# Atticuszz/GsplatLoc

Measured on AMD Instinct MI355X. Metric: Gaussians/s fwd+bwd @1M splats 1200x680, higher is better.
Workload: dtype f32

## Files before the change

### gsplatloc_amd/csrc/gsloc_common.h

```cpp
#pragma once
#include <hip/hip_runtime.h>
#include <stdint.h>

#include "../../include/gsloc_hip.h"

#define GSL_WAVE 64
#define GSL_ALPHA_MAX 0.999f
#define GSL_ALPHA_MIN (1.0f / 255.0f)
#define GSL_T_STOP 1e-4f
#define GSL_LOG2E 1.4426950408889634f

#define GSL_CHECK_LAUNCH()                                   \
  do {                                                       \
    hipError_t e__ = hipGetLastError();                      \
    if (e__ != hipSuccess) return GSL_ERR_HIP;               \
  } while (0)

namespace gsl {

int zero_u32(void* p, size_t n_dwords, hipStream_t st);

struct M3 {
  float m[9];
  __device__ __forceinline__ float& operator()(int r, int c) { return m[r * 3 + c]; }
// ... 42 lines not shown
  M3 R = quat_to_rotmat(q[0], q[1], q[2], q[3]);
  M3 M;
#pragma unroll
  for (int i = 0; i < 3; ++i)
#pragma unroll
    for (int j = 0; j < 3; ++j) M(i, j) = R(i, j) * s[j];
  return mul_bt(M, M);
}

struct Cam {
  M3 R;
  float t[3];
  float fx, fy, cx, cy;
};

__device__ __forceinline__ Cam load_cam(const float* __restrict__ V, const float* __restrict__ K) {
  Cam c;
#pragma unroll
  for (int i = 0; i < 3; ++i) {
#pragma unroll
    for (int j = 0; j < 3; ++j) c.R(i, j) = V[i * 4 + j];
    c.t[i] = V[i * 4 + 3];
  }
  c.fx = K[0]; c.fy = K[4]; c.cx = K[2]; c.cy = K[5];
  return c;
}

#define GSL_Q(arr, g) (arr)[(g)]
#ifndef GSL_NG
#define GSL_NG 4
#endif
#define GSL_HIT_SHIFT (32 - GSL_NG)
#define GSL_HIT_INDEX_MASK ((1u << GSL_HIT_SHIFT) - 1u)
#define GSL_CLAMP_DEPTH_WINDOW(nearp, farp)            \
  do {                                                 \
    if (!((nearp) >= 1.17549435e-38f)) (nearp) = 1.17549435e-38f; \
    if (!((farp) <= 3.40282347e+38f)) (farp) = 3.40282347e+38f;   \
  } while (0)
#define GSL_MAX_GAUSSIANS (1 << 26)
#ifndef GSL_XCD_SPANS
#define GSL_XCD_SPANS 0
#endif
__device__ __forceinline__ int xcd_span_item(int b, int n) {
#if GSL_XCD_SPANS
  const int x = b & 7, k = b >> 3, q = n >> 3, r = n & 7;
  return x * q + min(x, r) + k;
#else
  (void)n;
  return b;
#endif
}
#define GSL_TILE_OF_BLOCK() gsl::xcd_span_item((int)blockIdx.x, (int)gridDim.x)

__device__ __forceinline__ unsigned pack2h(float a, float b) {
  _Float16 ha = (_Float16)a, hb = (_Float16)b;
  return (unsigned)__builtin_bit_cast(unsigned short, ha) | ((unsigned)__builtin_bit_cast(unsigned short, hb) << 16);
}
__device__ __forceinline__ float h_lo(unsigned u) { return (float)__builtin_bit_cast(_Float16, (unsigned short)(u & 0xFFFFu)); }
__device__ __forceinline__ float h_hi(unsigned u) { return (float)__builtin_bit_cast(_Float16, (unsigned short)(u >> 16)); }

__device__ __forceinline__ void store_half_record(uint4* __restrict__ Qh, size_t i, float4 q0, float4 q1, float4 q2) {
  float rc = (q1.w > 0.f && q1.w < 6.0e4f) ? q1.w * 1.002f + 0.01f : q1.w;
  Qh[2 * i] = make_uint4(__float_as_uint(q0.x), __float_as_uint(q0.y), pack2h(q1.x, q1.y), pack2h(q1.z, rc));
  Qh[2 * i + 1] = make_uint4(pack2h(0.f, q0.w), pack2h(q2.x, q2.y), pack2h(q2.z, 0.f), __float_as_uint(q0.z));
}

// ... 349 lines not shown
```

### gsplatloc_amd/csrc/raster_g16.hip

```cpp
#include <stdlib.h>
#include <string.h>

#include "gsloc_common.h"

namespace gsl {

__device__ __forceinline__ float g16_sel(unsigned long long m, float t, float f) {
  float r;
  asm("v_cndmask_b32_e64 %0, %1, %2, %3" : "=v"(r) : "v"(f), "v"(t), "s"(m));
  return r;
}

#define G16_M_LO8 0x00FF00FF00FF00FFull
#define G16_M_B2 0x0F0F0F0F0F0F0F0Full
#define G16_M_B1 0x3333333333333333ull
#define G16_M_B0 0x5555555555555555ull

constexpr int G16_NG = GSL_NG;
constexpr int G16_GL = 64 / G16_NG;
static_assert(G16_NG == 4 || G16_NG == 8, "pixel groups are DPP rows or half rows");

__device__ __forceinline__ float row_scatter8(const float (&v)[8]) {
  float n0, n1, n2, n3, m0, m1;
  asm volatile(
// ... 48 lines not shown
      "v_add_f32_dpp %2, %6, %6 row_half_mirror row_mask:0xf bank_mask:0xf\n\t"
      "v_add_f32_dpp %3, %7, %7 row_half_mirror row_mask:0xf bank_mask:0xf\n\t"
      "v_add_f32_dpp %0, %8, %8 row_half_mirror row_mask:0xf bank_mask:0xa\n\t"
      "v_add_f32_dpp %1, %9, %9 row_half_mirror row_mask:0xf bank_mask:0xa\n\t"
      "v_add_f32_dpp %2, %10, %10 row_half_mirror row_mask:0xf bank_mask:0xa\n\t"
      "s_nop 1\n\t"
      : "=&v"(n0), "=&v"(n1), "=&v"(n2), "=&v"(n3)
      : "v"(v[0]), "v"(v[1]), "v"(v[2]), "v"(v[3]), "v"(v[4]), "v"(v[5]), "v"(v[6]));
  n0 += dpp_get<0x4E>(n0); n1 += dpp_get<0x4E>(n1); n2 += dpp_get<0x4E>(n2); n3 += dpp_get<0x4E>(n3);
  n0 += dpp_get<0xB1>(n0); n1 += dpp_get<0xB1>(n1); n2 += dpp_get<0xB1>(n2); n3 += dpp_get<0xB1>(n3);
  return make_float4(n0, n1, n2, n3);
}

__device__ __forceinline__ void half_scatter16(const float (&v)[16], float4& lo, float4& hi) {
  float a[8];
#pragma unroll
  for (int i = 0; i < 8; ++i) {
    float keep = g16_sel(G16_M_B2, v[i], v[i + 8]), send = g16_sel(G16_M_B2, v[i + 8], v[i]);
    a[i] = keep + dpp_get<0x141>(send);
  }
#pragma unroll
  for (int i = 0; i < 8; ++i) a[i] += dpp_get<0x4E>(a[i]);
#pragma unroll
  for (int i = 0; i < 8; ++i) a[i] += dpp_get<0xB1>(a[i]);
  lo = make_float4(a[0], a[1], a[2], a[3]);
  hi = make_float4(a[4], a[5], a[6], a[7]);
}

#ifdef GSL_G16_STATS
__device__ unsigned long long g16_stats[8];
#define G16_STAT(i, n) do { unsigned long long n__ = (unsigned long long)(n); if (lane == 0) atomicAdd(&g16_stats[i], n__); } while (0)
#else
#define G16_STAT(i, n) do { } while (0)
#endif

#ifndef GSL_QB
#define GSL_QB 64
#endif
#define GSL_QBS (GSL_QB + 1)
#ifndef GSL_Q_LCAP
#define GSL_Q_LCAP 24
#endif

template <int D, int CG>
struct QStage {
  static constexpr int NV = 6 + CG;
  static constexpr int NS = (NV <= 8) ? 8 : 16;
  static constexpr int A = 6 + D;
  static constexpr int LCAP = ((NS == 8) ? GSL_Q_LCAP : GSL_Q_LCAP / 2) * 4 / G16_NG;
  float4 s0[GSL_QBS];
  float4 s1[GSL_QBS];
  float4 s2[(D >= 3 && CG == D) ? GSL_QBS : 1];
  int32_t id[GSL_QBS];
  uint32_t posn[G16_NG / 4][GSL_QBS];
  alignas(16) float pair[G16_NG * LCAP * NS];
  uint8_t rlist[G16_NG][GSL_QBS + 4];
  uint8_t nzlist[64];
};

template <int D, int CG>
__device__ __forceinline__ void qraster_bwd_body(
    QStage<D, CG>& sb, const float4* __restrict__ Q0, const float4* __restrict__ Q1, const float4* __restrict__ Q2,
    const uint4* __restrict__ Qh, const int32_t* __restrict__ flatten_ids, float* __restrict__ vacc, long long rs,
    long long re, int lane, int quad, float px, float py, float tx0, float ty0, int bin_final, float T_init,
    float Bp_init, const float (&vc)[D], const uint32_t* __restrict__ qhits, int n_qhits) {
  constexpr bool RGB = D >= 3;
// ... 5 lines not shown
  constexpr int NG = G16_NG, GL = G16_GL;
  constexpr int PP = 12;
  static_assert(A <= PP && NG * LCAP * NS >= 64 * PP, "64 packed gradient rows reuse the pair slots");
  static_assert(GSL_QB < 127 && GSL_QB >= 64, "7-bit list positions with 127 reserved; a chunk appends up to 64 entries");
  const int grp = lane / GL, p = lane & (GL - 1);
  const float tcx = tx0 + 8.f, tcy = ty0 + 8.f;
  const float lx = px - tcx, ly = py - tcy;
  const float lxx = lx * lx, lxy = lx * ly, lyy = ly * ly;
  float T = T_init;
  float Bp = Bp_init;
  const int myslot = (NG == 8) ? (p >> 2) * (NS / 2) : ((NS == 8) ? (p >> 1) : p);
  const bool writer = (NG == 8) ? ((p & 3) == 0) : ((NS == 8) ? ((p & 1) == 0) : true);
  float* const mypair = &sb.pair[grp * LCAP * NS + myslot];
  uint8_t* const mylist = sb.rlist[grp];
  const unsigned long long lt = (1ull << lane) - 1ull;
  const float qx0 = tx0 + 8.f * (float)(quad & 1), qy0 = ty0 + 8.f * (float)(quad >> 1);
  int grp_final[NG];
  {
    int rf = bin_final;
    rf = max(rf, __shfl_xor(rf, 1, 64));
    rf = max(rf, __shfl_xor(rf, 2, 64));
    rf = max(rf, __shfl_xor(rf, 4, 64));
    if (GL == 16) rf = max(rf, __shfl_xor(rf, 8, 64));
#pragma unroll
    for (int g = 0; g < NG; ++g) grp_final[g] = __builtin_amdgcn_readlane(rf, GL * g);
  }
  if (lane == 0) {
    sb.s0[GSL_QB] = make_float4(0.f, 0.f, 0.f, 0.f);
    sb.s1[GSL_QB] = make_float4(0.f, 0.f, 0.f, 0.f);
    if (RGB && CG == D) sb.s2[GSL_QB] = make_float4(0.f, 0.f, 0.f, 0.f);
  }
  int pos = __builtin_amdgcn_readfirstlane(qhits ? n_qhits : (int)re);
  const int pos_end = __builtin_amdgcn_readfirstlane(qhits ? 0 : (int)rs);
  while (pos > pos_end) {
    int staged = 0;
    int cnt[NG];
#pragma unroll
    for (int g = 0; g < NG; ++g) cnt[g] = 0;
    __syncthreads();
    while (pos > pos_end && staged <= GSL_QB - 64) {
      long long idx = (long long)(pos - 1 - lane);
      bool in = idx >= (long long)pos_end;
      unsigned nib = 0;
      int gid = 0;
      float4 r0 = make_float4(0.f, 0.f, 0.f, 0.f), r1 = r0, r2 = r0;
      if (in) {
        if (qhits) {
          unsigned e = qhits[idx];
          nib = e >> GSL_HIT_SHIFT;
          idx = (long long)(e & GSL_HIT_INDEX_MASK);
          gid = flatten_ids[idx];
          load_record(Q0, Q1, Q2, Qh, gid, RGB && CG == D, r0, r1, r2);
        } else {
          gid = flatten_ids[idx];
          load_record(Q0, Q1, Q2, Qh, gid, RGB && CG == D, r0, r1, r2);
          if (r1.w >= 0.f) {
            float rr = r1.w * r1.w;
#pragma unroll
            for (int g = 0; g < NG; ++g) {
              const int b = (NG == 8) ? (g >> 1) : g;
              const float cy = (NG == 8) ? 2.f * (float)(g & 1) + 1.f : 2.f, hy = (NG == 8) ? 0.5f : 1.5f;
              float ex = fmaxf(fabsf(r0.x - (qx0 + 4.f * (float)(b & 1) + 2.f)) - 1.5f, 0.f);
              float ey = fmaxf(fabsf(r0.y - (qy0 + 4.f * (float)(b >> 1) + cy)) - hy, 0.f);
              bool h = (ex * ex + ey * ey <= rr) && ((int)idx <= grp_final[g]);
              nib |= (h ? 1u : 0u) << g;
            }
          }
        }
      }
      unsigned long long R = __ballot(nib != 0);
      int slot = staged + __popcll(R & lt);
      unsigned pack[NG / 4];
#pragma unroll
      for (int w = 0; w < NG / 4; ++w) pack[w] = 0x0FFFFFFFu;
#pragma unroll
      for (int g = 0; g < NG; ++g) {
        unsigned long long Bg = __ballot(nib & (1u << g));
        if (__builtin_amdgcn_inverse_ballot_w64(Bg)) {
          int q = cnt[g] + __popcll(Bg & lt);
          sb.rlist[g][q] = (uint8_t)slot;
          pack[g >> 2] ^= (127u ^ (unsigned)q) << (7 * (g & 3));
        }
        cnt[g] += __popcll(Bg);
      }
      if (__builtin_amdgcn_inverse_ballot_w64(R)) {
        sb.id[slot] = gid;
        sb.s0[slot] = r0;
        sb.s1[slot] = make_float4(r1.x * (0.5f * GSL_LOG2E), r1.y * GSL_LOG2E, r1.z * (0.5f * GSL_LOG2E),
                                  __int_as_float((int)idx));
        if (RGB && CG == D) sb.s2[slot] = r2;
#pragma unroll
        for (int w = 0; w < NG / 4; ++w) sb.posn[w][slot] = pack[w];
      }
      staged += __popcll(R);
      pos -= 64;
    }
    if (staged == 0) continue;
    int kmax = 0, cnt_tot = 0, cnt_my = 0;
#pragma unroll
    for (int g = 0; g < NG; ++g) {
      kmax = max(kmax, cnt[g]);
      cnt_tot += cnt[g];
      cnt_my = (grp == g) ? cnt[g] : cnt_my;
    }
    G16_STAT(6, kmax);
    G16_STAT(7, cnt_tot);
    (void)cnt_tot;
    for (int k = cnt_my + p; k < kmax + 3; k += GL) mylist[k] = (uint8_t)GSL_QB;
    __syncthreads();
    constexpr int NU = (GSL_QB + 63) / 64;
    float mo[NU][NV];
#pragma unroll
    for (int u = 0; u < NU; ++u)
#pragma unroll
      for (int q = 0; q < NV; ++q) mo[u][q] = 0.f;
    auto trip = [&](int t, const float4& c0, const float4& c1, float4& r, float4& r2) {
      float dx = c0.x - px, dy = c0.y - py;
      float sigma = fmaf(c1.y * dx, dy, fmaf(c1.x * dx, dx, c1.z * dy * dy));
      float vis = __builtin_amdgcn_exp2f(-sigma);
      float opv = c0.w * vis;
      float alpha = fminf(GSL_ALPHA_MAX, opv);
      unsigned long long validm = __ballot(__float_as_int(c1.w) <= bin_final) & __ballot(sigma >= 0.f) &
                                  __ballot(alpha >= GSL_ALPHA_MIN);
      G16_STAT(0, 1);
      r = make_float4(0.f, 0.f, 0.f, 0.f);
      r2 = r;
      if (validm) {
        G16_STAT(1, 1);
#ifdef GSL_G16_STATS
        {
          int groups_hit = 0;
          for (int g = 0; g < NG; ++g) groups_hit += ((validm >> (GL * g)) & ((1ull << GL) - 1ull)) != 0;
          G16_STAT(3, groups_hit);
        }
#endif
        G16_STAT(5, __popcll(validm));
        unsigned long long capm = __ballot(opv <= GSL_ALPHA_MAX);
        float am = g16_sel(validm, alpha, 0.f);
        float ra = __builtin_amdgcn_rcpf(1.f - am);
        T *= ra;
        float fac = am * T;
        float cdot;
// ... 29 lines not shown
          else r.x = row_scatter16(reinterpret_cast<const float(&)[16]>(val));
        }
      }
    };
    auto put = [&](float* dst, const float4& r, const float4& r2) {
      if (NG == 8) {
        *reinterpret_cast<float4*>(dst) = r;
        if (NS == 16) *reinterpret_cast<float4*>(dst + 4) = r2;
      } else {
        *dst = r.x;
      }
    };
    for (int k0 = 0; k0 < kmax; k0 += LCAP) {
      const int k1 = min(k0 + LCAP, kmax);
      int t0 = mylist[k0], t1 = mylist[k0 + 1];
      float4 qa0 = sb.s0[t0], qa1 = sb.s1[t0];
      float4 ra = make_float4(0.f, 0.f, 0.f, 0.f), ra2 = ra, rb = ra, rb2 = ra;
      float* dst = mypair;
      for (int k = k0; k < k1; k += 2) {
        if (k > k0 && writer) put(dst - NS, rb, rb2);
        const int t2 = mylist[k + 2];
        const float4 qb0 = sb.s0[t1], qb1 = sb.s1[t1];
        trip(t0, qa0, qa1, ra, ra2);
        if (writer) put(dst, ra, ra2);
        const int t3 = mylist[k + 3];
        qa0 = sb.s0[t2];
        qa1 = sb.s1[t2];
        trip(t1, qb0, qb1, rb, rb2);
        t0 = t2;
        t1 = t3;
        dst += 2 * NS;
      }
      if (writer) put(dst - NS, rb, rb2);
      __syncthreads();
#pragma unroll
      for (int u = 0; u < NU; ++u) {
        int slot = lane + 64 * u;
        if (slot < staged) {
#pragma unroll
          for (int w = 0; w < NG / 4; ++w) {
            unsigned pk = sb.posn[w][slot];
#pragma unroll
            for (int g4 = 0; g4 < 4; ++g4) {
              const int g = 4 * w + g4;
              const unsigned q = ((pk >> (7 * g4)) & 127u) - (unsigned)k0;
              if (q < (unsigned)LCAP) {
                const float4* src = reinterpret_cast<const float4*>(&sb.pair[(g * LCAP + q) * NS]);
                float4 a = src[0], c = src[1];
                mo[u][0] += a.x; mo[u][1] += a.y; mo[u][2] += a.z; mo[u][3] += a.w;
                mo[u][4] += c.x; mo[u][5] += c.y; mo[u][6] += c.z;
                if (NV > 7) mo[u][7 < NV ? 7 : 0] += c.w;
                if (NS == 16) {
                  float4 e = src[2];
                  if (NV > 8) mo[u][8 < NV ? 8 : 0] += e.x;
                  if (NV > 9) mo[u][9 < NV ? 9 : 0] += e.y;
                }
              }
            }
          }
        }
      }
      __syncthreads();
    }
#pragma unroll
    for (int u = 0; u < NU; ++u) {
      int slot = lane + 64 * u;
      bool nz = false;
      float row[A];
#pragma unroll
      for (int k = 0; k < A; ++k) row[k] = 0.f;
      if (slot < staged) {
        {
          unsigned bits = 0u;
#pragma unroll
          for (int k = 0; k < NV; ++k) bits |= __float_as_uint(mo[u][k]);
          nz = (bits << 1) != 0u;
        }
        if (nz) {
          float4 r0 = sb.s0[slot], r1 = sb.s1[slot];
          float X = r0.x - tcx, Y = r0.y - tcy, S = mo[u][0];
          float Sx = X * S - mo[u][1], Sy = Y * S - mo[u][2];
          float Sxx = X * (X * S - 2.f * mo[u][1]) + mo[u][3];
          float Sxy = X * (Y * S - mo[u][2]) - Y * mo[u][1] + mo[u][4];
          float Syy = Y * (Y * S - 2.f * mo[u][2]) + mo[u][5];
          float no = -r0.w;
          r1.x *= 2.f / GSL_LOG2E; r1.y *= 1.f / GSL_LOG2E; r1.z *= 2.f / GSL_LOG2E;
          row[0] = no * (r1.x * Sx + r1.y * Sy);
          row[1] = no * (r1.y * Sx + r1.z * Sy);
          row[2] = 0.5f * no * Sxx;
          row[3] = no * Sxy;
          row[4] = 0.5f * no * Syy;
          row[5] = S;
          if (CG == D) {
#pragma unroll
            for (int ch = 0; ch < D; ++ch) row[6 + ch] = mo[u][6 + ch];
          } else {
            row[6 + D - 1] = mo[u][6];
          }
        }
      }
      float* packed = sb.pair;
      if (nz) {
#pragma unroll
        for (int k = 0; k < A; ++k) packed[lane * PP + k] = row[k];
      }
      unsigned long long mask = __ballot(nz);
      int cntz = __popcll(mask);
      if (nz) sb.nzlist[__popcll(mask & lt)] = (uint8_t)lane;
      __syncthreads();
      constexpr int RPI = 64 / A;
      const int arow = lane / A, f = lane - arow * A;
      for (int i0 = 0; i0 < cntz; i0 += RPI) {
        int gi = i0 + arow;
        if (gi < cntz && arow < RPI) {
          int sl = sb.nzlist[gi];
          const unsigned off = ((unsigned)sb.id[sl + 64 * u] << 6) | ((unsigned)f << 2);
          atomicAdd(reinterpret_cast<float*>(reinterpret_cast<char*>(vacc) + off), packed[sl * PP + f]);
        }
      }
      __syncthreads();
    }
  }
}

template <int D, bool ED, int CG, bool LONG>
__device__ __forceinline__ void qraster_bwd_item(
    QStage<D, CG>& sb, int b, int n_items, const float4* __restrict__ Q0, const float4* __restrict__ Q1,
    const float4* __restrict__ Q2, int W, int H, int tile_w, int ty0, const int32_t* __restrict__ tile_offsets,
    const int32_t* __restrict__ flatten_ids, long long capacity, const float* __restrict__ render,
    const float* __restrict__ alphas, const int32_t* __restrict__ last_ids, const float* __restrict__ v_render,
    const float* __restrict__ v_alphas, float* __restrict__ vacc, int row0, int row1, const uint4* __restrict__ Qh,
    const uint32_t* __restrict__ isect_hits, int32_t* __restrict__ isect_hit_counts, int long_min, LongWs lw,
    int32_t* __restrict__ rgb_flag, int32_t* __restrict__ clear_counts, int32_t* __restrict__ clear_state) {
  if (!LONG && (CG == 1 || D == 3) && clear_counts && (b & 3) == 0 && threadIdx.x == 0) {
    clear_counts[ty0 * tile_w + (b >> 2)] = 0;
    if (b == 0 && clear_state) *clear_state = 0;
  }
  const int wi = LONG ? b : xcd_span_item(b, n_items);
  const int quad = wi & 3, item = wi >> 2;
  int tile, sgm = 0, gseg = 0;
  if (LONG) {
    gseg = item;
    if (gseg >= lw.n_seg[0]) return;
    tile = lw.seg_tile[gseg];
    sgm = lw.seg_idx[gseg];
    if (tile < 0) return;
  } else {
    tile = ty0 * tile_w + item;
  }
  int tyi = tile / tile_w, txi = tile - tyi * tile_w;
  int lane = threadIdx.x, grp = lane >> 4, p = lane & 15;
  int j = txi * 16 + (quad & 1) * 8 + (grp & 1) * 4 + (p & 3);
  int i = tyi * 16 + (quad >> 1) * 8 + (grp >> 1) * 4 + (p >> 2);
  float px = (float)j + 0.5f, py = (float)i + 0.5f;
  bool inside = (i < H) && (j < W) && (i >= row0) && (i < row1);
// ... 55 lines not shown
        for (int u = 0; u < 8; ++u) {
          if (stop || s0 + u >= nseg) continue;
          if (t8[u] == 2.f) { stop = true; continue; }
          float cc[4] = {c8[u].x, c8[u].y, c8[u].z, c8[u].w};
          float dot = 0.f;
#pragma unroll
          for (int k = 0; k < D; ++k) dot += vc[k] * cc[k];
          Bp_init += dot;
          if (t8[u] < 0.f) stop = true;
        }
      }
    }
  }
  const uint32_t* qh = nullptr;
  int nqh = 0;
  if (isect_hits) {
    long long ls = tile_offsets[tile], le = tile_offsets[tile + 1];
    if (le > capacity) le = capacity;
    if (LONG) {
      ls += (long long)sgm * GSL_SEG;
      le = min(ls + (long long)GSL_SEG, le);
      nqh = lw.seg_qcnt[gseg * 4 + quad];
    } else {
      nqh = isect_hit_counts[tile * 4 + quad];
    }
    qh = isect_hits + 4 * ls + (long long)quad * (le - ls);
    if (nqh == 0) return;
  }
  qraster_bwd_body<D, CG>(sb, Q0, Q1, Q2, Qh, flatten_ids, vacc, rs, re, lane, quad, px, py, (float)(txi * 16),
                          (float)(tyi * 16), bin_final, T_init, Bp_init, vc, qh, nqh);
}

template <int D, bool ED, int CG, bool LONG>
__global__ __launch_bounds__(64) void k_qraster_bwd(
    const float4* __restrict__ Q0, const float4* __restrict__ Q1, const float4* __restrict__ Q2, int W, int H,
    int tile_w, int ty0, const int32_t* __restrict__ tile_offsets, const int32_t* __restrict__ flatten_ids,
    long long capacity, const float* __restrict__ render, const float* __restrict__ alphas,
    const int32_t* __restrict__ last_ids, const float* __restrict__ v_render, const float* __restrict__ v_alphas,
    float* __restrict__ vacc, int row0, int row1, const uint4* __restrict__ Qh,
    const uint32_t* __restrict__ isect_hits, int32_t* __restrict__ isect_hit_counts, int long_min, LongWs lw,
    int32_t* __restrict__ rgb_flag, int32_t* __restrict__ clear_counts, int32_t* __restrict__ clear_state, int n_items) {
  __shared__ QStage<D, CG> sb;
  if (D == 4 && CG == D && rgb_flag && *rgb_flag == 0) return;
  for (int b = (int)blockIdx.x; b < n_items; b += (int)gridDim.x) {
    qraster_bwd_item<D, ED, CG, LONG>(sb, b, n_items, Q0, Q1, Q2, W, H, tile_w, ty0, tile_offsets, flatten_ids, capacity,
                                      render, alphas, last_ids, v_render, v_alphas, vacc, row0, row1, Qh, isect_hits,
                                      isect_hit_counts, long_min, lw, rgb_flag, clear_counts, clear_state);
    __syncthreads();
  }
}

}

#ifdef GSL_G16_STATS
extern "C" int gsl_g16_stats(unsigned long long* host_out, int reset) {
  if (hipMemcpyFromSymbol(host_out, HIP_SYMBOL(gsl::g16_stats), sizeof(unsigned long long) * 8) != hipSuccess) return -3;
  if (reset) {
    unsigned long long z[8] = {0};
    if (hipMemcpyToSymbol(HIP_SYMBOL(gsl::g16_stats), z, sizeof(z)) != hipSuccess) return -3;
  }
  return 0;
}
#endif

extern "C" int32_t* gsl_fused_bin_state(void* ws, int n_tiles);

extern "C" int gsl_g16_raster_bwd_launch(const float* Q0, const float* Q1, const float* Q2, int channels, int ed, int width,
                                         int height, int tile_w, int ty0, int ty1, const int32_t* tile_offsets,
                                         const int32_t* flatten_ids, int64_t capacity, const float* render,
                                         const float* alphas, const int32_t* last_ids, const float* v_render,
                                         const float* v_alphas, float* vacc, int row0, int row1, const void* Qh,
                                         const uint32_t* isect_hits, const int32_t* isect_hit_counts, int long_min,
                                         void* long_ws, int max_seg, int rgb_flag_index, void* clear_ws,
                                         void* stream) {
  hipStream_t st = (hipStream_t)stream;
  int nblk = long_ws ? max_seg : (ty1 - ty0) * tile_w;
  gsl::LongWs lw = gsl::long_ws_views(long_ws ? long_ws : (void*)0, long_ws ? max_seg : 0);
  const bool lng = long_ws != nullptr;
  int32_t* rgb_flag = isect_hit_counts ? const_cast<int32_t*>(isect_hit_counts) + rgb_flag_index : nullptr;
  int32_t* clear_counts = (int32_t*)clear_ws;
  int32_t* clear_state = clear_ws ? gsl_fused_bin_state(clear_ws, rgb_flag_index / 4) : nullptr;
#define CALL_Q(DD, EE, CC)                                                                                   \
  do {                                                                                                       \
    const int n_items = 4 * nblk;                                                                            \
    const int grid = ((DD) == 4 && (CC) == 4 && rgb_flag && n_items > 2048) ? 2048 : n_items;                \
    if (lng)                                                                                                 \
      hipLaunchKernelGGL((gsl::k_qraster_bwd<DD, EE, CC, true>), dim3(grid), dim3(64), 0, st, (const float4*)Q0, \
                         (const float4*)Q1, (const float4*)Q2, width, height, tile_w, ty0, tile_offsets,     \
                         flatten_ids, (long long)capacity, render, alphas, last_ids, v_render, v_alphas, vacc, \
                         row0, row1, (const uint4*)Qh, isect_hits, const_cast<int32_t*>(isect_hit_counts), long_min, lw, rgb_flag, clear_counts, clear_state, n_items);                   \
    else                                                                                                     \
      hipLaunchKernelGGL((gsl::k_qraster_bwd<DD, EE, CC, false>), dim3(grid), dim3(64), 0, st, (const float4*)Q0, \
// ... 16 lines not shown
```

### gsplatloc_amd/csrc/raster_px.hip

```cpp
#include "gsloc_common.h"
#include "loss_dev.h"
#include "sort_dev.h"

namespace gsl {

template <int D>
struct PStage {
  float4 s0[256];
  float4 s1[256];
  float4 s2[(D >= 3) ? 256 : 1];
  uint16_t qlist[4][256];
  int qcnt[4][4];
};

template <int SHIFT = 0, typename Stage>
__device__ __forceinline__ int compact_quadrants(Stage& sb, int tid, bool valid_rec, float x, float y, float r,
                                                 float tile_x0, float tile_y0) {
  int lane = tid & 63, wv = tid >> 6;
  unsigned long long B[4];
#pragma unroll
  for (int q = 0; q < 4; ++q) {
    float cx = tile_x0 + 4.f + 8.f * (float)(q & 1), cy = tile_y0 + 4.f + 8.f * (float)(q >> 1);
    B[q] = __ballot(valid_rec) & __ballot(fabsf(x - cx) <= r + 3.5f) & __ballot(fabsf(y - cy) <= r + 3.5f);
  }
  if (lane < 4) {
    unsigned long long b = lane == 0 ? B[0] : (lane == 1 ? B[1] : (lane == 2 ? B[2] : B[3]));
    sb.qcnt[wv][lane] = __popcll(b);
  }
  __syncthreads();
  unsigned long long lt = (1ull << lane) - 1ull;
#pragma unroll
  for (int q = 0; q < 4; ++q) {
    if ((B[q] >> lane) & 1ull) {
      int base = 0;
      for (int w = 0; w < wv; ++w) base += sb.qcnt[w][q];
      sb.qlist[q][base + __popcll(B[q] & lt)] = (uint16_t)(tid << SHIFT);
    }
// ... 52 lines not shown
  return r;
}

__device__ __forceinline__ int ffbl_raw(unsigned v) {
  int r;
  asm("v_ffbl_b32 %0, %1" : "=v"(r) : "v"(v));
  return r;
}

__device__ __forceinline__ float4 rec_at(const float4* arr, unsigned off) {
  return *reinterpret_cast<const float4*>(reinterpret_cast<const char*>(arr) + off);
}

__device__ __forceinline__ void box_range(float centre_rel, float r, int& lo, int& hi) {
  float l = ceilf(centre_rel - r), h = floorf(centre_rel + r);
  lo = (int)fmaxf(l, 0.f);
  hi = (int)fminf(h, 7.f);
}

template <int D, int MODE>
__device__ __forceinline__ void praster_walk(
    PStage<D>& sb, const float4* __restrict__ Q0, const float4* __restrict__ Q1, const float4* __restrict__ Q2,
    const uint4* __restrict__ Qh, const int32_t* __restrict__ flatten_ids, long long rs, long long re, int tid, float px,
    float py, int qx, int qy, int txi, int tyi, bool& done, float& T, float (&pix)[D], int& cur_idx,
    uint32_t* __restrict__ isect_hits, int& n_hits) {
  constexpr bool RGB = D >= 3;
  constexpr bool DEPTH = (D == 1) || (D == 4);
  const int lane = tid & 63, wv = tid >> 6;
  int nb = (int)((re - rs + 255) / 256);
  if (MODE == 1) isect_hits = nullptr;
  uint32_t* const qout = isect_hits ? isect_hits + 4 * rs + (long long)wv * (re - rs) : nullptr;
  n_hits = 0;
  unsigned long long DONE = __ballot(done);
  for (int b = 0; b < nb; ++b) {
    if (__syncthreads_and(DONE == ~0ull)) break;
    long long bstart = rs + (long long)b * 256;
    int bsize = (int)min((long long)256, re - bstart);
    float4 r0 = make_float4(0.f, 0.f, 0.f, 0.f), r1 = make_float4(0.f, 0.f, 0.f, -1.f);
    if (tid < bsize) {
      int g = flatten_ids[bstart + tid];
      float4 r2 = make_float4(0.f, 0.f, 0.f, 0.f);
      load_record(Q0, Q1, Q2, Qh, g, RGB && MODE == 0, r0, r1, r2);
      const float ca = r1.x * (0.5f * GSL_LOG2E), cb = r1.y * GSL_LOG2E, cc = r1.z * (0.5f * GSL_LOG2E);
      sb.s0[tid] = make_float4(r0.x, r0.y, ca, cb);
      if (RGB) {
        sb.s1[tid] = make_float4(cc, r0.w, r2.x, r2.y);
        sb.s2[tid] = make_float4(r2.z, r0.z, r1.w, 0.f);
      } else {
        sb.s1[tid] = make_float4(cc, r0.w, r0.z, r1.w);
      }
    } else {
      sb.s0[tid] = make_float4(0.f, 0.f, 0.f, 0.f);
      if (RGB) {
        sb.s1[tid] = make_float4(0.f, 0.f, 0.f, 0.f);
        sb.s2[tid] = make_float4(0.f, 0.f, -1.f, 0.f);
      } else {
        sb.s1[tid] = make_float4(0.f, 0.f, 0.f, -1.f);
      }
    }
    const int n = __builtin_amdgcn_readfirstlane(
        compact_quadrants<4>(sb, tid, tid < bsize, r0.x, r0.y, r1.w, (float)(txi * 16), (float)(tyi * 16)));
    for (int c = 0; c < n; c += 64) {
      if (DONE == ~0ull) break;
      int e = c + lane;
      int lox = 1, hix = 0, loy = 1, hiy = 0;
      if (e < n) {
        const unsigned off = sb.qlist[wv][e];
        float4 a0 = rec_at(sb.s0, off);
        float r = RGB ? rec_at(sb.s2, off).z : rec_at(sb.s1, off).w;
        box_range(a0.x - ((float)qx + 0.5f), r, lox, hix);
        box_range(a0.y - ((float)qy + 0.5f), r, loy, hiy);
      }
      unsigned mlo, mhi;
      pixel_masks<true>(lox, hix, loy, hiy, lane, mlo, mhi);
      mlo = sel_u32(DONE, 0u, mlo);
      mhi = sel_u32(DONE, 0u, mhi);
      unsigned cm[2] = {0u, 0u};
#pragma unroll
      for (int half = 0; half < 2; ++half) {
        unsigned m = half ? mhi : mlo;
        if (half) m = sel_u32(DONE, 0u, m);
        const uint16_t* const ql = &sb.qlist[wv][c + half * 32];
        unsigned long long ACT = __ballot(m != 0);
        if (ACT) do {
          const unsigned b0 = m & (0u - m);
          m ^= b0;
          const unsigned b1 = m & (0u - m);
          m ^= b1;
          const unsigned long long TWO = __ballot(b1 != 0u);
          const unsigned t0 = ql[ffbl_raw(b0)] & 0xFF0u;
          const unsigned t1 = ql[ffbl_raw(b1)] & 0xFF0u;
          float4 p0 = rec_at(sb.s0, t0), p1 = rec_at(sb.s1, t0);
          float4 u0 = rec_at(sb.s0, t1), u1 = rec_at(sb.s1, t1);
          float dx0 = p0.x - px, dy0 = p0.y - py, dx1 = u0.x - px, dy1 = u0.y - py;
          float sg0 = fmaf(p0.w * dx0, dy0, fmaf(p0.z * dx0, dx0, p1.x * dy0 * dy0));
          float sg1 = fmaf(u0.w * dx1, dy1, fmaf(u0.z * dx1, dx1, u1.x * dy1 * dy1));
          float al0 = fminf(GSL_ALPHA_MAX, p1.y * __builtin_amdgcn_exp2f(-sg0));
          float al1 = fminf(GSL_ALPHA_MAX, u1.y * __builtin_amdgcn_exp2f(-sg1));
          const unsigned long long OK0 = ACT & __ballot(sg0 >= 0.f) & __ballot(al0 >= GSL_ALPHA_MIN);
          const unsigned long long OK1 = TWO & __ballot(sg1 >= 0.f) & __ballot(al1 >= GSL_ALPHA_MIN);
          if (MODE == 1) {
            T *= 1.f - sel_f32(OK0, al0, 0.f);
            T *= 1.f - sel_f32(OK1, al1, 0.f);
            ACT = __ballot(m != 0);
            continue;
          }
          const unsigned long long S0R = __ballot(T * (1.f - al0) <= GSL_T_STOP);
          const unsigned long long STOP0 = OK0 & S0R, EFF0 = OK0 & ~S0R;
          const float a0 = sel_f32(EFF0, al0, 0.f);
          const float vis0 = a0 * T;
          const float T1 = T * (1.f - a0);
          const unsigned long long LIVE1 = OK1 & ~STOP0;
          const unsigned long long S1R = __ballot(T1 * (1.f - al1) <= GSL_T_STOP);
          const unsigned long long STOP1 = LIVE1 & S1R, EFF1 = LIVE1 & ~S1R;
          const float a1 = sel_f32(EFF1, al1, 0.f);
          const float vis1 = a1 * T1;
          T = T1 * (1.f - a1);
          if (RGB) {
            const float2 q20 = *reinterpret_cast<const float2*>(reinterpret_cast<const char*>(sb.s2) + t0);
            const float2 q21 = *reinterpret_cast<const float2*>(reinterpret_cast<const char*>(sb.s2) + t1);
            pix[0] += p1.z * vis0; pix[1] += p1.w * vis0; pix[2] += q20.x * vis0;
            if (DEPTH) pix[D - 1] += q20.y * vis0;
            pix[0] += u1.z * vis1; pix[1] += u1.w * vis1; pix[2] += q21.x * vis1;
            if (DEPTH) pix[D - 1] += q21.y * vis1;
          } else if (DEPTH) {
            pix[D - 1] += p1.z * vis0;
            pix[D - 1] += u1.z * vis1;
          }
          cm[half] |= sel_u32(EFF0, b0, 0u) | sel_u32(EFF1, b1, 0u);
          const unsigned long long STOPPED = STOP0 | STOP1;
          DONE |= STOPPED;
          m = sel_u32(STOPPED, 0u, m);
          ACT = __ballot(m != 0);
        } while (ACT);
      }
      {
        const bool any = (cm[0] | cm[1]) != 0u;
        const int pos = cm[1] ? 63 - __clz((int)cm[1]) : 31 - __clz((int)(cm[0] | 1u));
        const int tl = (sb.qlist[wv][c + pos] & 0xFF0u) >> 4;
        cur_idx = any ? (int)bstart + tl : cur_idx;
      }
      if (isect_hits) {
        unsigned rlo = group_or(cm[0]), rhi = group_or(cm[1]);
        unsigned nib = 0;
        unsigned long long Rm = 0ull;
#pragma unroll
        for (int g = 0; g < GSL_NG; ++g) {
          unsigned glo = (unsigned)__builtin_amdgcn_readlane((int)rlo, (64 / GSL_NG) * g);
          unsigned ghi = (unsigned)__builtin_amdgcn_readlane((int)rhi, (64 / GSL_NG) * g);
          unsigned long long gm = ((unsigned long long)ghi << 32) | glo;
          nib |= sel_u32(gm, 1u << g, 0u);
          Rm |= gm;
        }
        if (nib) qout[n_hits + __popcll(Rm & ((1ull << lane) - 1ull))] = (nib << GSL_HIT_SHIFT) | (unsigned)((int)bstart + (sb.qlist[wv][e] >> 4));
        n_hits += __popcll(Rm);
      }
    }
  }
  done = ((DONE >> lane) & 1ull) != 0ull;
}

struct TilePixel {
  int tyi, txi, qx, qy, i, j;
};
__device__ __forceinline__ TilePixel tile_pixel(int tile, int tile_w, int tid) {
  TilePixel t;
  int lane = tid & 63, wv = tid >> 6, grp = lane >> 4, pp = lane & 15;
  t.tyi = tile / tile_w;
  t.txi = tile - t.tyi * tile_w;
  t.qx = t.txi * 16 + (wv & 1) * 8;
  t.qy = t.tyi * 16 + (wv >> 1) * 8;
  t.j = t.qx + 4 * (grp & 1) + (pp & 3);
  t.i = t.qy + 4 * (grp >> 1) + (pp >> 2);
  return t;
}

struct FwdSort {
  uint64_t* bins;
  const int32_t* counts;
  int32_t* tile_offsets;
  int32_t* flatten_ids;
  int32_t* n_isects;
  int32_t* flags;
  int bin_cap;
  const int32_t* storage_of;
};
template <int SORT> struct FwdListPtr { typedef const int32_t* __restrict__ type; };
template <> struct FwdListPtr<2> { typedef const int32_t* type; };
template <> struct FwdListPtr<3> { typedef const int32_t* type; };

template <int D, bool ED, int SORT>
__global__ __launch_bounds__(256) __attribute__((amdgpu_waves_per_eu(SORT == 3 ? 4 : 6))) void k_praster_fwd(
    const float4* __restrict__ Q0, const float4* __restrict__ Q1, const float4* __restrict__ Q2, int W, int H,
    int tile_w, int ty0, typename FwdListPtr<SORT>::type tile_offsets, typename FwdListPtr<SORT>::type flatten_ids,
    long long capacity, float* __restrict__ render, float* __restrict__ alphas, int32_t* __restrict__ last_ids,
    int row0, int row1, const uint4* __restrict__ Qh, int32_t* __restrict__ clear_counts,
    int32_t* __restrict__ clear_state, uint32_t* __restrict__ isect_hits, int32_t* __restrict__ isect_hit_counts,
    int long_min, int n_tiles_total, FwdSort fs) {
  constexpr size_t SORT_BYTES = SORT ? (size_t)8 * 64 * (1 << SORT) * sizeof(uint64_t) : 0;
  constexpr size_t LDS_BYTES = sizeof(PStage<D>) > SORT_BYTES ? sizeof(PStage<D>) : SORT_BYTES;
  __shared__ __align__(16) unsigned char smem[LDS_BYTES];
  PStage<D>& sb = *reinterpret_cast<PStage<D>*>(smem);
  __shared__ int s_scan[5];
  int tile = ty0 * tile_w + GSL_TILE_OF_BLOCK();
  long long sorted_rs = 0, sorted_re = 0;
  if constexpr (SORT != 0) {
    const int tid = threadIdx.x, lane = tid & 63, wv = tid >> 6;
    int acc = prefix_count_share(fs.counts, tile, fs.bin_cap, tid);
#pragma unroll
    for (int o = 32; o >= 1; o >>= 1) acc += __shfl_xor(acc, o, 64);
    if (lane == 0) s_scan[wv] = acc;
    if (tid == 0) {
      int c_own = fs.counts[tile];
      s_scan[4] = min(c_own, fs.bin_cap);
      if (c_own > fs.bin_cap && fs.flags) { fs.flags[1] = 1; atomicMax(&fs.flags[2], c_own); }
    }
    __syncthreads();
    long long s0 = s_scan[0] + s_scan[1] + s_scan[2] + s_scan[3], e0 = s0 + s_scan[4];
    if (tid == 0) {
      fs.tile_offsets[tile] = (int32_t)s0;
      if (tile == n_tiles_total - 1) {
        fs.tile_offsets[tile + 1] = (int32_t)e0;
        if (fs.n_isects) fs.n_isects[0] = (int32_t)e0;
      }
    }
    if (e0 > capacity) e0 = capacity;
    int n = (int)max(e0 - s0, (long long)0);
    if (n > 256) {
      wg_sort_tile<SORT>(fs.bins + (size_t)tile * (size_t)fs.bin_cap, n, s0, tile, tid, reinterpret_cast<uint64_t*>(smem),
                         nullptr, fs.flatten_ids, nullptr, 0, fs.storage_of);
    } else if (n > 0 && wv == 0) {
      const uint64_t* src = fs.bins + (size_t)tile * (size_t)fs.bin_cap;
      uint64_t k[4];
#pragma unroll
      for (int r = 0; r < 4; ++r) k[r] = (lane * 4 + r < n) ? src[lane * 4 + r] : GSL_SORT_PAD;
      wave_sort_regs<2>(k, lane);
// ... 17 lines not shown
  bool inside = (i < H) && (j < W) && (i >= row0) && (i < row1);
  bool done = !inside;

  long long rs, re;
  if constexpr (SORT != 0) {
    rs = sorted_rs;
    re = sorted_re;
  } else {
    rs = tile_offsets[tile];
    re = tile_offsets[tile + 1];
    if (re > capacity) re = capacity;
    if (rs > re) rs = re;
    if (long_min > 0 && re - rs > long_min) return;
  }

  float T = 1.f;
  int cur_idx = 0;
  float pix[D];
#pragma unroll
  for (int k = 0; k < D; ++k) pix[k] = 0.f;
  int n_hits = 0;
  praster_walk<D, 0>(sb, Q0, Q1, Q2, Qh, flatten_ids, rs, re, tid, px, py, tp.qx, tp.qy, tp.txi, tp.tyi, done, T, pix,
                     cur_idx, isect_hits, n_hits);
  if (isect_hits && (tid & 63) == 0) isect_hit_counts[tile * 4 + (tid >> 6)] = n_hits;
  if (inside) {
    size_t pid = (size_t)i * W + j;
    float A = 1.f - T;
    alphas[pid] = A;
    if (ED) pix[D - 1] = pix[D - 1] / fmaxf(A, 1e-10f);
#pragma unroll
    for (int k = 0; k < D; ++k) render[pid * D + k] = pix[k];
    last_ids[pid] = cur_idx;
  }
}

template <int D, int PASS>
__global__ __launch_bounds__(256) void k_long_fwd(
    const float4* __restrict__ Q0, const float4* __restrict__ Q1, const float4* __restrict__ Q2, int W, int H,
    int tile_w, const int32_t* __restrict__ tile_offsets, const int32_t* __restrict__ flatten_ids, long long capacity,
    int row0, int row1, const uint4* __restrict__ Qh, uint32_t* __restrict__ isect_hits, LongWs w) {
  __shared__ PStage<D> sb;
  int g = blockIdx.x;
  if (g >= w.n_seg[0]) return;
  int tile = w.seg_tile[g], sgm = w.seg_idx[g];
  if (tile < 0) return;
  int tid = threadIdx.x;
  TilePixel tp = tile_pixel(tile, tile_w, tid);
  int i = tp.i, j = tp.j;
  float px = (float)j + 0.5f, py = (float)i + 0.5f;
  bool inside = (i < H) && (j < W) && (i >= row0) && (i < row1);
  long long rs = tile_offsets[tile], re = tile_offsets[tile + 1];
  if (re > capacity) re = capacity;
  long long ss = rs + (long long)sgm * GSL_SEG, se = min(ss + (long long)GSL_SEG, re);
  float pix[D];
#pragma unroll
  for (int k = 0; k < D; ++k) pix[k] = 0.f;
  size_t slot = (size_t)g * 256 + tid;
  if (PASS == 0) {
    float T = 1.f;
    int cur = 0;
    bool done = !inside;
    int nh = 0;
    praster_walk<D, 1>(sb, Q0, Q1, Q2, Qh, flatten_ids, ss, se, tid, px, py, tp.qx, tp.qy, tp.txi, tp.tyi, done, T, pix,
                       cur, nullptr, nh);
    w.P[slot] = T;
  } else {
// ... 274 lines not shown
          const float T1 = T0 * ra1;
          const float fac1 = a1 * T1;
          const float va1 = T1 * cd1 - ra1 * Bp0;
          T = T1;
          Bp = Bp0 + fac1 * cd1;
          if (__builtin_amdgcn_inverse_ballot_w64(OK0)) {
            float w = (opv0 <= GSL_ALPHA_MAX) ? vis0 * va0 : 0.f;
            int cc = j - tiny_origin(p0.x, p1.w), rr = i - tiny_origin(p0.y, p1.w);
            if ((unsigned)cc < 4u && (unsigned)rr < 4u)
              trec[(size_t)sb.id[t0] * 16 + rr * 4 + cc] = make_float2(w, fac0);
            else if (flags)
              flags[0] = 1;
          }
          if (__builtin_amdgcn_inverse_ballot_w64(OK1)) {
            float w = (opv1 <= GSL_ALPHA_MAX) ? vis1 * va1 : 0.f;
            int cc = j - tiny_origin(u0.x, u1.w), rr = i - tiny_origin(u0.y, u1.w);
            if ((unsigned)cc < 4u && (unsigned)rr < 4u)
              trec[(size_t)sb.id[t1] * 16 + rr * 4 + cc] = make_float2(w, fac1);
            else if (flags)
              flags[0] = 1;
          }
          ACT = __ballot(m != 0);
        } while (ACT);
      }
    }
  }
}


}

extern "C" int32_t* gsl_fused_bin_state(void* ws, int n_tiles);

extern "C" int gsl_tiny_raster_bwd(const float* Q0, const float* Q1, const float* Q2, int channels, int ed, int width,
                                   int height, int tile_w, int tile_h, int ty0, int ty1, const int32_t* tile_offsets,
                                   const int32_t* flatten_ids, int64_t capacity, const float* render,
                                   const float* alphas, const int32_t* last_ids, const float* v_render,
                                   const float* v_alphas, float* trec, float* vcT, int row0, int row1,
                                   int32_t* flags, int long_min, const float* loss_depth_gt, float depth_lambda,
                                   float edge_lambda, float* loss_partials, void* clear_ws, void* stream) {
  if (width <= 0 || height <= 0 || tile_w <= 0 || tile_h <= 0 || ty0 < 0 || ty1 > tile_h || ty0 > ty1 ||
      capacity < 0 || row0 < 0 || row0 > row1)
    return GSL_ERR_BAD_ARG;
  if (tile_w * 16 < width || tile_h * 16 < height) return GSL_ERR_BAD_ARG;
  if (!tile_offsets || !render || !alphas || !last_ids || !v_render || !v_alphas || !trec || !vcT)
    return GSL_ERR_BAD_ARG;
  if (ed && channels == 3) return GSL_ERR_BAD_ARG;
  const bool loss = loss_depth_gt != nullptr;
  if (loss && (!loss_partials || ty0 != 0 || ty1 != tile_h || row0 != 0 || row1 < height ||
               tile_w != (width + 15) / 16 || tile_h != (height + 15) / 16 || (channels != 1 && channels != 4)))
    return GSL_ERR_BAD_ARG;
  if (ty0 == ty1) return GSL_OK;
  if (capacity > 0 && (!Q0 || !Q1 || !flatten_ids || (channels >= 3 && !Q2))) return GSL_ERR_BAD_ARG;
  hipStream_t st = (hipStream_t)stream;
  int nblk = (ty1 - ty0) * tile_w;
  gsl::TinyLoss tl{loss_depth_gt, loss_partials, const_cast<float*>(v_render), depth_lambda, edge_lambda,
                   1.0f / ((float)width * (float)height)};
#define CALL_TB(DD, EE, LL)                                                                                  \
  hipLaunchKernelGGL((gsl::k_tiny_bwd<DD, EE, LL>), dim3(nblk), dim3(256), 0, st, (const float4*)Q0,        \
                     (const float4*)Q1, (const float4*)Q2, width, height, tile_w, ty0, tile_offsets,         \
                     flatten_ids, (long long)capacity, render, alphas, last_ids, v_render, v_alphas,         \
                     (float2*)trec, vcT, row0, row1, flags, long_min, tl, (int32_t*)clear_ws,                \
                     clear_ws ? gsl_fused_bin_state(clear_ws, tile_w * tile_h) : (int32_t*)nullptr)
#define CALL_TL(DD, EE) do { if (loss) CALL_TB(DD, EE, true); else CALL_TB(DD, EE, false); } while (0)
  if (channels == 1) { if (ed) CALL_TL(1, true); else CALL_TL(1, false); }
  else if (channels == 3) { CALL_TB(3, false, false); }
// ... 107 lines not shown
```

Before: 2.370 billion.

## Prefetch next staging batch records during qraster backward compute and raise waves per EU

In the quad-raster backward pass, the first 64-entry staging load of each batch (hit word, flatten id, and Gaussian record) is now issued early in three steps spread across the previous batch's compute phases. The aim is to hide global memory latency behind the LDS/compute work. The kernel also gains an amdgpu_waves_per_eu attribute (5 or 6) to push for higher occupancy, at the risk of register spills given the extra live prefetch registers. Optional wall-clock phase instrumentation is added behind GSL_PHASE_STATS.

```diff
diff --git a/gsplatloc_amd/csrc/gsloc_common.h b/gsplatloc_amd/csrc/gsloc_common.h
--- a/gsplatloc_amd/csrc/gsloc_common.h
+++ b/gsplatloc_amd/csrc/gsloc_common.h
@@ -98,6 +98,28 @@
 #endif
 #define GSL_HIT_SHIFT (32 - GSL_NG)
 #define GSL_HIT_INDEX_MASK ((1u << GSL_HIT_SHIFT) - 1u)
+#ifdef GSL_PHASE_STATS
+#define GSL_PH_DECL(n) unsigned long long ph_acc__[n] = {}; unsigned long long ph_t__ = wall_clock64()
+#define GSL_PH(k)                                  \
+  do {                                             \
+    const unsigned long long t__ = wall_clock64(); \
+    ph_acc__[k] += t__ - ph_t__;                   \
+    ph_t__ = t__;                                  \
+  } while (0)
+#define GSL_PH_COUNT(k) (ph_acc__[k] += 1ull)
+#define GSL_PH_WAIT() asm volatile("s_waitcnt vmcnt(0)" ::: "memory")
+#define GSL_PH_FLUSH(arr, n)                                                     \
+  do {                                                                           \
+    if ((threadIdx.x & 63) == 0)                                                 \
+      for (int k__ = 0; k__ < (n); ++k__) atomicAdd(&(arr)[k__], ph_acc__[k__]); \
+  } while (0)
+#else
+#define GSL_PH_DECL(n) do { } while (0)
+#define GSL_PH(k) do { } while (0)
+#define GSL_PH_COUNT(k) do { } while (0)
+#define GSL_PH_WAIT() do { } while (0)
+#define GSL_PH_FLUSH(arr, n) do { } while (0)
+#endif
 #define GSL_CLAMP_DEPTH_WINDOW(nearp, farp)            \
   do {                                                 \
     if (!((nearp) >= 1.17549435e-38f)) (nearp) = 1.17549435e-38f; \
diff --git a/gsplatloc_amd/csrc/raster_g16.hip b/gsplatloc_amd/csrc/raster_g16.hip
--- a/gsplatloc_amd/csrc/raster_g16.hip
+++ b/gsplatloc_amd/csrc/raster_g16.hip
@@ -104,6 +104,18 @@
 #define G16_STAT(i, n) do { unsigned long long n__ = (unsigned long long)(n); if (lane == 0) atomicAdd(&g16_stats[i], n__); } while (0)
 #else
 #define G16_STAT(i, n) do { } while (0)
+#endif
+
+#ifdef GSL_PHASE_STATS
+__device__ unsigned long long qbwd_phase[8];
+#endif
+
+#ifndef GSL_Q_PREFETCH
+#define GSL_Q_PREFETCH 1
+#endif
+
+#ifndef GSL_Q_MIN_WAVES
+#define GSL_Q_MIN_WAVES(D, CG) (((D) == 4 && (CG) == 4) ? 5 : 6)
 #endif
 
 #ifndef GSL_QB
@@ -175,28 +187,72 @@
   }
   int pos = __builtin_amdgcn_readfirstlane(qhits ? n_qhits : (int)re);
   const int pos_end = __builtin_amdgcn_readfirstlane(qhits ? 0 : (int)rs);
+  GSL_PH_DECL(6);
+  unsigned pf_w = 0u;
+  int pf_gid = 0;
+  float4 pf_r0 = make_float4(0.f, 0.f, 0.f, 0.f), pf_r1 = pf_r0, pf_r2 = pf_r0;
+  auto pf_in = [&]() { return pos - 1 - lane >= pos_end; };
+  auto pf_word = [&]() {
+    pf_w = 0u;
+    if (pf_in()) pf_w = qhits ? qhits[pos - 1 - lane] : (unsigned)flatten_ids[pos - 1 - lane];
+  };
+  auto pf_id = [&]() {
+    pf_gid = 0;
+    if (pf_in()) pf_gid = qhits ? flatten_ids[pf_w & GSL_HIT_INDEX_MASK] : (int)pf_w;
+  };
+  auto pf_record = [&]() {
+    pf_r0 = make_float4(0.f, 0.f, 0.f, 0.f);
+    pf_r1 = pf_r0;
+    pf_r2 = pf_r0;
+    if (pf_in()) load_record(Q0, Q1, Q2, Qh, pf_gid, RGB && CG == D, pf_r0, pf_r1, pf_r2);
+  };
+  if (GSL_Q_PREFETCH && pos > pos_end) {
+    pf_word();
+    pf_id();
+    pf_record();
+  }
   while (pos > pos_end) {
     int staged = 0;
     int cnt[NG];
 #pragma unroll
     for (int g = 0; g < NG; ++g) cnt[g] = 0;
     __syncthreads();
+    bool first = true;
     while (pos > pos_end && staged <= GSL_QB - 64) {
+      GSL_PH(1);
       long long idx = (long long)(pos - 1 - lane);
       bool in = idx >= (long long)pos_end;
       unsigned nib = 0;
       int gid = 0;
       float4 r0 = make_float4(0.f, 0.f, 0.f, 0.f), r1 = r0, r2 = r0;
-      if (in) {
+      if (GSL_Q_PREFETCH && first) {
+        if (in) {
+          if (qhits) {
+            nib = pf_w >> GSL_HIT_SHIFT;
+            idx = (long long)(pf_w & GSL_HIT_INDEX_MASK);
+          }
+          gid = pf_gid;
+          r0 = pf_r0;
+          r1 = pf_r1;
+          r2 = pf_r2;
+        }
+      } else if (in) {
         if (qhits) {
           unsigned e = qhits[idx];
           nib = e >> GSL_HIT_SHIFT;
           idx = (long long)(e & GSL_HIT_INDEX_MASK);
           gid = flatten_ids[idx];
-          load_record(Q0, Q1, Q2, Qh, gid, RGB && CG == D, r0, r1, r2);
         } else {
           gid = flatten_ids[idx];
-          load_record(Q0, Q1, Q2, Qh, gid, RGB && CG == D, r0, r1, r2);
+        }
+        load_record(Q0, Q1, Q2, Qh, gid, RGB && CG == D, r0, r1, r2);
+      }
+      first = false;
+      GSL_PH_WAIT();
+      GSL_PH(0);
+      GSL_PH_COUNT(4);
+      if (in) {
+        if (!qhits) {
           if (r1.w >= 0.f) {
             float rr = r1.w * r1.w;
 #pragma unroll
@@ -238,7 +294,9 @@
       staged += __popcll(R);
       pos -= 64;
     }
+    if (GSL_Q_PREFETCH) pf_word();
     if (staged == 0) continue;
+    GSL_PH_COUNT(5);
     int kmax = 0, cnt_tot = 0, cnt_my = 0;
 #pragma unroll
     for (int g = 0; g < NG; ++g) {
@@ -251,6 +309,7 @@
     (void)cnt_tot;
     for (int k = cnt_my + p; k < kmax + 3; k += GL) mylist[k] = (uint8_t)GSL_QB;
     __syncthreads();
+    GSL_PH(1);
     constexpr int NU = (GSL_QB + 63) / 64;
     float mo[NU][NV];
 #pragma unroll
@@ -346,7 +405,9 @@
         dst += 2 * NS;
       }
       if (writer) put(dst - NS, rb, rb2);
+      if (GSL_Q_PREFETCH && k0 == 0) pf_id();
       __syncthreads();
+      GSL_PH(2);
 #pragma unroll
       for (int u = 0; u < NU; ++u) {
         int slot = lane + 64 * u;
@@ -375,7 +436,9 @@
         }
       }
       __syncthreads();
+      GSL_PH(3);
     }
+    if (GSL_Q_PREFETCH) pf_record();
 #pragma unroll
     for (int u = 0; u < NU; ++u) {
       int slot = lane + 64 * u;
@@ -434,7 +497,9 @@
       }
       __syncthreads();
     }
-  }
+    GSL_PH(3);
+  }
+  GSL_PH_FLUSH(qbwd_phase, 6);
 }
 
 template <int D, bool ED, int CG, bool LONG>
@@ -556,7 +621,7 @@
 }
 
 template <int D, bool ED, int CG, bool LONG>
-__global__ __launch_bounds__(64) void k_qraster_bwd(
+__global__ __launch_bounds__(64) __attribute__((amdgpu_waves_per_eu(GSL_Q_MIN_WAVES(D, CG)))) void k_qraster_bwd(
     const float4* __restrict__ Q0, const float4* __restrict__ Q1, const float4* __restrict__ Q2, int W, int H,
     int tile_w, int ty0, const int32_t* __restrict__ tile_offsets, const int32_t* __restrict__ flatten_ids,
     long long capacity, const float* __restrict__ render, const float* __restrict__ alphas,
@@ -567,9 +632,15 @@
   __shared__ QStage<D, CG> sb;
   if (D == 4 && CG == D && rgb_flag && *rgb_flag == 0) return;
   for (int b = (int)blockIdx.x; b < n_items; b += (int)gridDim.x) {
+#ifdef GSL_PHASE_STATS
+    const unsigned long long t_item = wall_clock64();
+#endif
     qraster_bwd_item<D, ED, CG, LONG>(sb, b, n_items, Q0, Q1, Q2, W, H, tile_w, ty0, tile_offsets, flatten_ids, capacity,
                                       render, alphas, last_ids, v_render, v_alphas, vacc, row0, row1, Qh, isect_hits,
                                       isect_hit_counts, long_min, lw, rgb_flag, clear_counts, clear_state);
+#ifdef GSL_PHASE_STATS
+    if (threadIdx.x == 0) atomicAdd(&qbwd_phase[7], wall_clock64() - t_item);
+#endif
     __syncthreads();
   }
 }
@@ -582,6 +653,21 @@
   if (reset) {
     unsigned long long z[8] = {0};
     if (hipMemcpyToSymbol(HIP_SYMBOL(gsl::g16_stats), z, sizeof(z)) != hipSuccess) return -3;
+  }
+  return 0;
+}
+#endif
+
+#ifdef GSL_PHASE_STATS
+extern "C" int gsl_qbwd_phase_stats(unsigned long long* host_out, int reset) {
+  if (hipMemcpyFromSymbol(host_out, HIP_SYMBOL(gsl::qbwd_phase), sizeof(unsigned long long) * 8) != hipSuccess) return -3;
+  int dev = 0, khz = 0;
+  if (hipGetDevice(&dev) != hipSuccess || hipDeviceGetAttribute(&khz, hipDeviceAttributeWallClockRate, dev) != hipSuccess)
+    return -3;
+  host_out[8] = (unsigned long long)khz;
+  if (reset) {
+    unsigned long long z[8] = {0};
+    if (hipMemcpyToSymbol(HIP_SYMBOL(gsl::qbwd_phase), z, sizeof(z)) != hipSuccess) return -3;
   }
   return 0;
 }
diff --git a/gsplatloc_amd/csrc/raster_px.hip b/gsplatloc_amd/csrc/raster_px.hip
--- a/gsplatloc_amd/csrc/raster_px.hip
+++ b/gsplatloc_amd/csrc/raster_px.hip
@@ -3,6 +3,10 @@
 #include "sort_dev.h"
 
 namespace gsl {
+
+#ifdef GSL_PHASE_STATS
+__device__ unsigned long long pfwd_phase[8];
+#endif
 
 template <int D>
 struct PStage {
@@ -121,8 +125,12 @@
   uint32_t* const qout = isect_hits ? isect_hits + 4 * rs + (long long)wv * (re - rs) : nullptr;
   n_hits = 0;
   unsigned long long DONE = __ballot(done);
+  GSL_PH_DECL(7);
   for (int b = 0; b < nb; ++b) {
+    GSL_PH(5);
     if (__syncthreads_and(DONE == ~0ull)) break;
+    GSL_PH(0);
+    GSL_PH_COUNT(6);
     long long bstart = rs + (long long)b * 256;
     int bsize = (int)min((long long)256, re - bstart);
     float4 r0 = make_float4(0.f, 0.f, 0.f, 0.f), r1 = make_float4(0.f, 0.f, 0.f, -1.f);
@@ -147,9 +155,13 @@
         sb.s1[tid] = make_float4(0.f, 0.f, 0.f, -1.f);
       }
     }
+    GSL_PH_WAIT();
+    GSL_PH(1);
     const int n = __builtin_amdgcn_readfirstlane(
         compact_quadrants<4>(sb, tid, tid < bsize, r0.x, r0.y, r1.w, (float)(txi * 16), (float)(tyi * 16)));
+    GSL_PH(2);
     for (int c = 0; c < n; c += 64) {
+      GSL_PH(5);
       if (DONE == ~0ull) break;
       int e = c + lane;
       int lox = 1, hix = 0, loy = 1, hiy = 0;
@@ -164,6 +176,7 @@
       pixel_masks<true>(lox, hix, loy, hiy, lane, mlo, mhi);
       mlo = sel_u32(DONE, 0u, mlo);
       mhi = sel_u32(DONE, 0u, mhi);
+      GSL_PH(3);
       unsigned cm[2] = {0u, 0u};
 #pragma unroll
       for (int half = 0; half < 2; ++half) {
@@ -223,6 +236,7 @@
           ACT = __ballot(m != 0);
         } while (ACT);
       }
+      GSL_PH(4);
       {
         const bool any = (cm[0] | cm[1]) != 0u;
         const int pos = cm[1] ? 63 - __clz((int)cm[1]) : 31 - __clz((int)(cm[0] | 1u));
@@ -246,6 +260,8 @@
       }
     }
   }
+  GSL_PH(5);
+  GSL_PH_FLUSH(pfwd_phase, 7);
   done = ((DONE >> lane) & 1ull) != 0ull;
 }
 
@@ -291,6 +307,9 @@
   __shared__ __align__(16) unsigned char smem[LDS_BYTES];
   PStage<D>& sb = *reinterpret_cast<PStage<D>*>(smem);
   __shared__ int s_scan[5];
+#ifdef GSL_PHASE_STATS
+  const unsigned long long t_kernel = wall_clock64();
+#endif
   int tile = ty0 * tile_w + GSL_TILE_OF_BLOCK();
   long long sorted_rs = 0, sorted_re = 0;
   if constexpr (SORT != 0) {
@@ -374,6 +393,9 @@
     for (int k = 0; k < D; ++k) render[pid * D + k] = pix[k];
     last_ids[pid] = cur_idx;
   }
+#ifdef GSL_PHASE_STATS
+  if ((threadIdx.x & 63) == 0) atomicAdd(&pfwd_phase[7], wall_clock64() - t_kernel);
+#endif
 }
 
 template <int D, int PASS>
@@ -714,6 +736,21 @@
 
 extern "C" int32_t* gsl_fused_bin_state(void* ws, int n_tiles);
 
+#ifdef GSL_PHASE_STATS
+extern "C" int gsl_pfwd_phase_stats(unsigned long long* host_out, int reset) {
+  if (hipMemcpyFromSymbol(host_out, HIP_SYMBOL(gsl::pfwd_phase), sizeof(unsigned long long) * 8) != hipSuccess) return -3;
+  int dev = 0, khz = 0;
+  if (hipGetDevice(&dev) != hipSuccess || hipDeviceGetAttribute(&khz, hipDeviceAttributeWallClockRate, dev) != hipSuccess)
+    return -3;
+  host_out[8] = (unsigned long long)khz;
+  if (reset) {
+    unsigned long long z[8] = {0};
+    if (hipMemcpyToSymbol(HIP_SYMBOL(gsl::pfwd_phase), z, sizeof(z)) != hipSuccess) return -3;
+  }
+  return 0;
+}
+#endif
+
 extern "C" int gsl_tiny_raster_bwd(const float* Q0, const float* Q1, const float* Q2, int channels, int ed, int width,
                                    int height, int tile_w, int tile_h, int ty0, int ty1, const int32_t* tile_offsets,
                                    const int32_t* flatten_ids, int64_t capacity, const float* render,
```

Result: no change. 2.384 billion (median of 6 runs) (+0.6%).
